# granne/granne

Measured on AMD Instinct MI355X. Metric: queries/sec (recall@10 alongside), 10M x 100-d angular, batch=1024, higher is better.
Workload: dtype f32; 1 GPU; C2 (BASELINE.json configs[1]): 10000000 x 100-d f32 angular, i.i.d. uniform components, batch=1024, ef_search=50, k=10; n_elements=10000000, dim=100, batch=1024, ef_search=50, k=10

## Files before the change

granne_amd/_lib.py:

```python
import ctypes as C
import os

from . import build as _build

F32, I8, F16 = 0, 1, 2
UNUSED = 0xFFFFFFFF
BUILD_ALL = 0xFFFFFFFFFFFFFFFF

OK = 0
ERR_INVALID, ERR_HIP, ERR_NO_DEVICE, ERR_OVERFLOW, ERR_IO = -1, -2, -3, -4, -5

OPT_VISITED_SLOTS, OPT_FORCE_SLOW, OPT_SLOW_SLOTS, OPT_SLOW_BLOCKS, OPT_OVERFLOW_SLOTS = 1, 2, 3, 4, 5
OPT_VISITED16, OPT_VISITED16_LG, OPT_LAST_WALKER, OPT_SEARCH_DEPTH, OPT_INLINE_TAILS, OPT_SEEN_MIN = 6, 7, 8, 9, 10, 11
OPT_SKETCH = 12
OPT_COALESCE, OPT_COALESCE_MAX, OPT_COALESCE_WAIT_US, OPT_COALESCED_LAUNCHES, OPT_COALESCED_QUERIES = 13, 14, 15, 16, 17
OPT_LAST_COMPACT_ROWS = 18
OPT_LAST_SPLIT_TAIL = 19
OPT_LAST_SCAN = 20
OPT_FORCE_GENERAL = 21
(SCAN_NONE, SCAN_RING, SCAN_I8, SCAN_I8_CHUNKED, SCAN_B16_7_4, SCAN_B16_13_2, SCAN_B16_16_1, SCAN_B16_CHUNKED, SCAN_F32_52_4,
 SCAN_F32_100_2, SCAN_F32_128_1) = range(11)
EXACT_TOPK_KMAX = 1024
EXACT_TOPK_CAP = 4096
PF_MAX_STAGES = 8
# ... 54 lines not shown
    "granne_hip_index_create": (i32, [C.POINTER(vp), vp, u64, u32, i32, u32, vp, vp, vp, i32]),
    "granne_hip_index_create_csr": (i32, [C.POINTER(vp), vp, u64, u32, i32, u32, vp, vp, vp, i32]),
    "granne_hip_index_create_device": (i32, [C.POINTER(vp), vp, u64, u32, i32, u32, vp, vp, vp, i32, vp]),
    "granne_hip_index_destroy": (None, [vp]),
    "granne_hip_index_len": (u64, [vp]),
    "granne_hip_index_num_elements": (u64, [vp]),
    "granne_hip_index_num_layers": (u32, [vp]),
    "granne_hip_index_layer_len": (u64, [vp, u32]),
    "granne_hip_index_dim": (u32, [vp]),
    "granne_hip_index_dtype": (i32, [vp]),
    "granne_hip_index_device": (i32, [vp]),
    "granne_hip_index_hbm_bytes": (u64, [vp]),
    "granne_hip_index_get_neighbors": (i32, [vp, u64, u32, vp, u32, C.POINTER(u32)]),
    "granne_hip_index_get_element": (i32, [vp, u64, vp]),
    "granne_hip_index_get_sketch": (i32, [vp, u64, u64, vp]),
    "granne_hip_search_batch": (i32, [vp, vp, u32, u32, u32, vp, vp, vp, vp]),
    "granne_hip_search_batch_device": (i32, [vp, vp, u32, u32, u32, vp, vp, vp, vp, vp, vp]),
    "granne_hip_search_batches_device": (i32, [vp, u32, vp, u32, u32, u32, vp, vp, vp, vp, vp, vp]),
    "granne_hip_search_begin_device": (i32, [vp, vp, u32, u32, u32, vp, vp, vp, vp, vp, vp, C.POINTER(u64)]),
    "granne_hip_search_end_device": (i32, [vp, u64, vp]),
    "granne_hip_device_malloc": (i32, [C.POINTER(vp), u64, i32]),
    "granne_hip_device_free": (i32, [vp, i32]),
    "granne_hip_copy_to_device": (i32, [vp, vp, u64, i32, vp]),
    "granne_hip_copy_to_host": (i32, [vp, vp, u64, i32, vp]),
    "granne_hip_stream_create": (i32, [C.POINTER(vp), i32]),
    "granne_hip_stream_destroy": (i32, [vp, i32]),
    "granne_hip_stream_synchronize": (i32, [vp, i32]),
    "granne_hip_event_create": (i32, [vp]),
    "granne_hip_event_destroy": (None, [vp]),
    "granne_hip_event_elapsed_ms": (i32, [vp, vp, vp]),
# ... 171 lines not shown
```

granne_amd/csrc/brute_force.h:

```cpp
#pragma once

#include "util_kernels.h"

namespace granne_hip {

typedef float bf_f32x16 __attribute__((ext_vector_type(16)));
typedef int bf_i32x16 __attribute__((ext_vector_type(16)));
typedef int bf_i32x4 __attribute__((ext_vector_type(4)));

#ifndef GRANNE_BF_EXP
#define GRANNE_BF_EXP 0
#endif
#ifndef GRANNE_BF_SUB
#define GRANNE_BF_SUB 2
#endif
constexpr uint32_t BF_I8_SUB = GRANNE_BF_SUB;
constexpr uint32_t BF_QT = 256;
constexpr uint32_t BF_THREADS = 512;
constexpr uint32_t BF_EXTRA = 6;
constexpr uint32_t BF_KMAX = 16;

struct BfGeometry {
    uint32_t rows, qt, threads, lds;
};
// ... 1 lines not shown
struct BruteParams {
    const uint8_t* elements;
    uint64_t n;
    uint32_t row_bytes, row_stride, dim;
    const uint8_t* queries;
    uint32_t nq, kk;
    uint64_t per_range;
    uint64_t* part_ids;
    float* part_d;
    uint32_t* part_c;
    const float* inv_norm;
    const float* inv_gmax;
    const float* tau_in;
    uint32_t* share_hist;
    const uint8_t* qpad;
};

struct BfBlock { uint32_t qt, range; };
__device__ __forceinline__ BfBlock bf_block() {
    const uint32_t nqt = gridDim.x, G = gridDim.y;
    const uint32_t L = blockIdx.y * nqt + blockIdx.x;
    BfBlock b;
    if ((G & 7u) == 0u) {
        const uint32_t xcd = L & 7u, slot = L >> 3;
        b.range = xcd * (G >> 3) + slot / nqt;
        b.qt = slot % nqt;
    } else {
        b.qt = blockIdx.x;
        b.range = blockIdx.y;
    }
// ... 223 lines not shown
    if constexpr (PRIME) bf_write_max(P, best, blk.range, q, qlive, h);
    else bf_write_list(P, L, blk.range, q, qlive, h);
}

template <int KH, int R>
constexpr BfGeometry bf_f32_geometry() {
    constexpr uint32_t ET = 32u * R, STRIDE = 2u * KH + 4u;
    return {ET, BF_QT, BF_THREADS, ET * STRIDE * 4u};
}

typedef __bf16 bf_b16x8 __attribute__((ext_vector_type(8)));
typedef __bf16 bf_b16x4 __attribute__((ext_vector_type(4)));
#ifndef GRANNE_BF_B16_AHEAD
#define GRANNE_BF_B16_AHEAD 1
#endif
constexpr uint32_t BF_B16_THREADS = 512, BF_B16_QT = 256;
template <int KG, int R, bool PRIME = false>
__global__ __launch_bounds__(BF_B16_THREADS) void bf_b16_kernel(const BruteParams P) {
    extern __shared__ __align__(16) uint8_t smem_bf[];
    constexpr uint32_t ET = 32u * R;
    constexpr uint32_t COMPS = 16u * KG;
    constexpr uint32_t STRIDE_B = 2u * COMPS + 16u;
    uint8_t* tile_hi = smem_bf;
    uint8_t* tile_lo = smem_bf + (size_t)ET * STRIDE_B;
    const uint32_t tid = threadIdx.x, lane = tid & 63u, wave = tid >> 6;
    const uint32_t col = lane & 31u, h = lane >> 5;
    const BfBlock blk = bf_block();
    const uint32_t q = blk.qt * BF_B16_QT + wave * 32u + col;
    const bool qlive = q < P.nq;

    bf_b16x8 qh[KG], ql[KG];
// ... 939 lines not shown
__global__ void inv_gmax_kernel(const float* __restrict__ inv_norm, uint64_t n, float* __restrict__ out) {
    const uint64_t total = ((n + 31u) >> 5) * 2u;
    for (uint64_t t = (uint64_t)blockIdx.x * blockDim.x + threadIdx.x; t < total; t += (uint64_t)gridDim.x * blockDim.x) {
        const uint64_t b = t >> 1;
        const uint32_t h = (uint32_t)(t & 1u);
        float m = 0.0f;
        for (uint32_t g = 0; g < 4; ++g)
            for (uint32_t i = 0; i < 4; ++i) {
                const uint64_t row = b * 32u + 8u * g + 4u * h + i;
                if (row < n) m = __builtin_fmaxf(m, inv_norm[row]);
            }
        out[t] = m;
    }
}

__global__ __launch_bounds__(64) void bf_tau_kernel(const float* __restrict__ maxima, uint32_t ranges, uint32_t nq, uint32_t kk, float* __restrict__ tau) {
    const uint32_t q = blockIdx.x, lane = threadIdx.x;
    if (q >= nq) return;
    if (ranges < kk || ranges > 64u) {
        if (lane == 0u) tau[q] = -3.0e38f;
        return;
    }
    const float v = lane < ranges ? maxima[(size_t)lane * nq + q] : -3.0e38f;
    uint32_t rank = 0;
    for (uint32_t j = 0; j < ranges; ++j) {
        const float o = __uint_as_float((uint32_t)__builtin_amdgcn_readlane((int)__float_as_uint(v), (int)j));
        rank += (o > v || (o == v && j < lane)) ? 1u : 0u;
    }
    if (lane < ranges && rank + 1u == kk) tau[q] = v > -1.0e38f ? v - 2.0e-6f : -3.0e38f;
}
// ... 43 lines not shown
```

granne_amd/csrc/granne_hip.hip:

```cpp
#include <hip/hip_runtime.h>

#include <atomic>
#include <chrono>
#include <cstdarg>
#include <cstdio>
#include <cstdlib>
#include <cstring>
#include <memory>
#include <mutex>
#include <string>
#include <type_traits>
#include <vector>

#include "../../include/granne_hip.h"
#include "search_kernel.h"
#include "walk_fast.h"
#include "slow_kernel.h"
#include "util_kernels.h"
#include "brute_force.h"
#include "exact_topk.h"
#include "combiner.h"
#include "dev_mem.h"

using namespace granne_hip;
// ... 45 lines not shown
extern "C" const char* granne_hip_last_error(void) { return g_last_error.c_str(); }
extern "C" int granne_hip_abi_version(void) { return GRANNE_HIP_ABI_VERSION; }
extern "C" int granne_hip_device_count(int* out_count) {
    if (!out_count) return fail(GRANNE_HIP_ERR_INVALID, "out_count is null");
    int n = 0;
    hipError_t e = hipGetDeviceCount(&n);
    if (e != hipSuccess) {
        *out_count = 0;
        return fail(GRANNE_HIP_ERR_NO_DEVICE, "hipGetDeviceCount: %s", hipGetErrorString(e));
    }
    *out_count = n;
    return GRANNE_HIP_OK;
}

struct EnvKnobs {
    int visited = 0, touch_max = -1, inline_tails = 1, seen_min = -1, bf_b16 = 1, bf_ring = 1, sketch = 1, compact_rows = 1;
    EnvKnobs() {
        auto geti = [](const char* name, int dflt) {
            const char* e = getenv(name);
            return e ? atoi(e) : dflt;
        };
        visited = geti("GRANNE_HIP_VISITED", 0);
        inline_tails = geti("GRANNE_HIP_INLINE_TAILS", 1);
        bf_ring = geti("GRANNE_HIP_BF_RING", 1);
        bf_b16 = geti("GRANNE_HIP_BF_B16", 1);
        seen_min = geti("GRANNE_HIP_SEEN_MIN", -1);
        touch_max = geti("GRANNE_HIP_TOUCH_MAX", -1);
        compact_rows = geti("GRANNE_HIP_COMPACT_ROWS", 1);
        sketch = geti("GRANNE_HIP_SKETCH", 1);
    }
};
static const EnvKnobs& knobs() {
    static const EnvKnobs k;
    return k;
}

struct ScratchCache {
    struct Block {
        hipStream_t stream;
        DevBuf p;
// ... 52 lines not shown
    uint64_t opt_slow_slots = 1u << 18;
    uint64_t opt_slow_blocks = 16;
    uint64_t opt_overflow_slots = 0;
    uint64_t opt_visited16 = 0;
    uint64_t opt_visited16_lg = 0;
    uint64_t opt_inline_tails = 1;
    uint64_t opt_seen_min = 2048;
    uint64_t opt_sketch = 1;
    std::atomic<uint64_t> last_slow_count{0};
    std::atomic<uint64_t> last_walker{0};
    std::atomic<uint64_t> last_compact{0};
    std::atomic<uint64_t> last_split{0};
    std::atomic<uint64_t> last_scan{0};
    std::mutex norm_mu;
    DevBuf d_inv_norm;
    DevBuf d_sketch;
    struct HostCall {
        hipStream_t stream = nullptr;
        DevBuf d_buf;
        PinBuf h_pin;
    };
    std::mutex call_mu;
    std::vector<HostCall*> call_free;
    uint64_t opt_coalesce = 0;
    Combiner combiner;
    HostCall* group_call[Combiner::DEPTH] = {};
    ScratchCache scratch;
    struct Flight {
        hipStream_t stream = nullptr;
        hipEvent_t ready = nullptr, done = nullptr;
// ... 425 lines not shown
    if (ix->se) return se_rows_to_host(*ix->se, idx, 1, 1, (float*)out);
    DeviceGuard g(ix->device);
    HIP_TRY(hipMemcpy(out, ix->d_elements.as<uint8_t>() + idx * ix->row_stride, (size_t)ix->dim * elem_size(ix->dtype),
                      hipMemcpyDeviceToHost));
    return GRANNE_HIP_OK;
}

extern "C" int granne_hip_index_get_sketch(const granne_hip_index* ix, uint64_t first, uint64_t count, void* out) {
    if (!ix || (!out && count)) return fail(GRANNE_HIP_ERR_INVALID, "null argument");
    GRANNE_HIP_COMPACT_UNSUPPORTED(ix, "get_sketch");
    if (!ix->d_sketch) return fail(GRANNE_HIP_ERR_INVALID, "the index holds no row sketches");
    if (first > ix->n_elements || count > ix->n_elements - first) return fail(GRANNE_HIP_ERR_INVALID, "rows out of range");
    if (count == 0) return GRANNE_HIP_OK;
    DeviceGuard g(ix->device);
    HIP_TRY(hipMemcpy(out, ix->d_sketch.as<uint8_t>() + first * SKETCH_LINE, (size_t)count * SKETCH_LINE, hipMemcpyDeviceToHost));
    return GRANNE_HIP_OK;
}

extern "C" int granne_hip_index_set_option(granne_hip_index* ix, int option, uint64_t value) {
    if (!ix) return fail(GRANNE_HIP_ERR_INVALID, "index is null");
    switch (option) {
    case GRANNE_HIP_OPT_VISITED_SLOTS:
        {
            const uint64_t odd = value ? value >> __builtin_ctzll(value) : 1;
            if (value != 0 && (value < 256 || value > 32768 || (odd != 1 && odd != 3)))
                return fail(GRANNE_HIP_ERR_INVALID, "visited slots must be 0, 2^k or 3 * 2^k in [256, 32768]");
        }
        ix->opt_visited_slots = value;
        return GRANNE_HIP_OK;
    case GRANNE_HIP_OPT_FORCE_SLOW:
// ... 1184 lines not shown
    if (nq && m == 0) return GRANNE_HIP_OK;
    return dists_launch(ix, d_queries, nullptr, m ? m : 1, d_ids, (uint64_t)nq * m, d_out, d_status, stream);
}

static int merge_launch(const uint8_t* ids, const uint8_t* dists, const uint8_t* counts, uint64_t ids_stride,
                        uint64_t dists_stride, uint64_t counts_stride, const uint64_t* shard_offsets, uint32_t n_shards,
                        uint32_t nq, uint32_t k, uint64_t* d_out_ids, float* d_out_dists, uint32_t* d_out_counts,
                        int device_id, void* stream);

struct ScanPlan {
    uint64_t form;
    void (*fn)(const BruteParams);
    void (*prime)(const BruteParams);
    BfGeometry geo, prime_geo;
    uint64_t max_ranges = 64;
};
static ScanPlan plan_scan(const granne_hip_index* ix, uint32_t nq) {
    if (ix->dtype == GRANNE_HIP_I8) {
        if (ix->row_bytes > 128u)
            return {GRANNE_HIP_SCAN_I8_CHUNKED, bf_i8_chunked_kernel<4>, bf_i8_chunked_kernel<4, true>, bf_i8_chunked_geometry<4>(), bf_i8_chunked_geometry<4>()};
        if (knobs().bf_ring && ix->row_bytes == 128u && ix->row_stride == 128u && ix->n_elements < (1ull << 29)) {
            ScanPlan P{GRANNE_HIP_SCAN_RING, bf_i8_ring_kernel, bf_i8_kernel<4, true>, bf_ring_geometry(), bf_i8_geometry<4>()};
            if ((uint64_t)((nq + P.geo.qt - 1) / P.geo.qt) * 64u < 256u) P.max_ranges = 128;
            return P;
        }
        return {GRANNE_HIP_SCAN_I8, bf_i8_kernel<4>, bf_i8_kernel<4, true>, bf_i8_geometry<4>(), bf_i8_geometry<4>()};
    }
    if (knobs().bf_b16 && ix->dim <= 112) return {GRANNE_HIP_SCAN_B16_7_4, bf_b16_kernel<7, 4>, bf_b16_kernel<7, 4, true>, bf_b16_geometry<7, 4>(), bf_b16_geometry<7, 4>()};
    if (knobs().bf_b16 && ix->dim <= 208) return {GRANNE_HIP_SCAN_B16_13_2, bf_b16_kernel<13, 2>, bf_b16_kernel<13, 2, true>, bf_b16_geometry<13, 2>(), bf_b16_geometry<13, 2>()};
    if (ix->dim > 256) return {GRANNE_HIP_SCAN_B16_CHUNKED, bf_b16_chunked_kernel<2>, bf_b16_chunked_kernel<2, true>, bf_b16_chunked_geometry<2>(), bf_b16_chunked_geometry<2>()};
    if (knobs().bf_b16) return {GRANNE_HIP_SCAN_B16_16_1, bf_b16_kernel<16, 1>, bf_b16_kernel<16, 1, true>, bf_b16_geometry<16, 1>(), bf_b16_geometry<16, 1>()};
    if (ix->dim <= 104) return {GRANNE_HIP_SCAN_F32_52_4, bf_f32_kernel<52, 4>, bf_f32_kernel<52, 4, true>, bf_f32_geometry<52, 4>(), bf_f32_geometry<52, 4>()};
    if (ix->dim <= 200) return {GRANNE_HIP_SCAN_F32_100_2, bf_f32_kernel<100, 2>, bf_f32_kernel<100, 2, true>, bf_f32_geometry<100, 2>(), bf_f32_geometry<100, 2>()};
    return {GRANNE_HIP_SCAN_F32_128_1, bf_f32_kernel<128, 1>, bf_f32_kernel<128, 1, true>, bf_f32_geometry<128, 1>(), bf_f32_geometry<128, 1>()};
}

namespace {
struct ScanScratch {
    size_t pid, pd, pc, mid, md, mc, cand, ex, tau, share, qpad, total = 0;
    ScanScratch(uint64_t ranges, uint32_t nq, uint32_t kk, size_t share_bytes, size_t qpad_bytes) {
        auto take = [&](size_t bytes, size_t align) {
            total = (total + align - 1) & ~(align - 1);
            total += bytes;
// ... 84 lines not shown
        std::lock_guard<std::mutex> lk(mix->norm_mu);
        if (!mix->d_inv_norm) {
            DevBuf norms;
            HIP_TRY(norms.alloc((size_t)inv_norm_bytes(n)));
            float* dn = norms.as<float>();
            hipLaunchKernelGGL(inv_norm_rows_kernel, dim3(grid_for(n * 8, 256)), dim3(256), 0, s, ix->d_elements.as<uint8_t>(), n, ix->row_stride, dn);
            hipLaunchKernelGGL(inv_gmax_kernel, dim3(grid_for(n_pad / 16 + 1, 256)), dim3(256), 0, s, (const float*)dn, n, dn + n_pad);
            if (hipGetLastError() != hipSuccess || hipStreamSynchronize(s) != hipSuccess)
                return fail(GRANNE_HIP_ERR_HIP, "inv_norm_rows_kernel failed");
            mix->d_inv_norm = std::move(norms);
            mix->hbm_bytes += inv_norm_bytes(n);
        }
        P.inv_norm = mix->d_inv_norm.as<float>();
        P.inv_gmax = P.inv_norm + n_pad;
    }
    P.elements = ix->d_elements.as<uint8_t>();
    P.n = n;
    P.row_bytes = ix->row_bytes;
    P.row_stride = ix->row_stride;
    P.dim = ix->dim;
    P.queries = (const uint8_t*)d_queries;
    P.nq = nq;
    P.kk = kk;
    P.per_range = per_range;
    P.part_ids = (uint64_t*)(scratch + o.pid);
    P.part_d = (float*)(scratch + o.pd);
    P.part_c = (uint32_t*)(scratch + o.pc);
    if (S.geo.lds > 64u * 1024u) HIP_TRY(hipFuncSetAttribute((const void*)S.fn, hipFuncAttributeMaxDynamicSharedMemorySize, (int)S.geo.lds));
    P.tau_in = nullptr;
    P.share_hist = nullptr;
    P.qpad = nullptr;
    if (qpad_bytes) {
        hipLaunchKernelGGL(bf_pad_queries_kernel, dim3(grid_for(qpad_bytes, 256)), dim3(256), 0, s, (const uint8_t*)d_queries, nq, ix->dim,
                           ix->row_bytes, scratch + o.qpad);
        HIP_TRY(hipGetLastError());
        P.qpad = scratch + o.qpad;
    }
    if (primed) {
        BruteParams Q = P;
        Q.n = prime_n;
        Q.per_range = prime_per;
        const BfGeometry& pg = S.prime_geo;
        if (pg.lds > 64u * 1024u) HIP_TRY(hipFuncSetAttribute((const void*)S.prime, hipFuncAttributeMaxDynamicSharedMemorySize, (int)pg.lds));
        hipLaunchKernelGGL(S.prime, dim3((nq + pg.qt - 1) / pg.qt, (uint32_t)Gs), dim3(pg.threads), pg.lds, s, Q);
        HIP_TRY(hipGetLastError());
        hipLaunchKernelGGL(bf_tau_kernel, dim3(nq), dim3(64), 0, s, (const float*)P.part_d, (uint32_t)Gs, nq, kk, (float*)(scratch + o.tau));
        HIP_TRY(hipGetLastError());
        P.tau_in = (const float*)(scratch + o.tau);
        HIP_TRY(hipMemsetAsync(scratch + o.share, 0, share_bytes, s));
        P.share_hist = (uint32_t*)(scratch + o.share);
    }
    hipLaunchKernelGGL(S.fn, dim3((nq + S.geo.qt - 1) / S.geo.qt, (uint32_t)G), dim3(S.geo.threads), S.geo.lds, s, P);
    HIP_TRY(hipGetLastError());
    int rc = merge_ranges(P, (uint32_t)G, nq, kk, (uint64_t*)(scratch + o.mid), (float*)(scratch + o.md), (uint32_t*)(scratch + o.mc),
                          ix->device, stream);
    if (rc) return rc;
    const uint32_t pairs = nq * kk;
    hipLaunchKernelGGL(bf_narrow_ids_kernel, dim3((pairs + 255) / 256), dim3(256), 0, s, (const uint64_t*)(scratch + o.mid),
                       (const uint32_t*)(scratch + o.mc), nq, kk, (uint32_t*)(scratch + o.cand));
    HIP_TRY(hipGetLastError());
    rc = dists_launch(ix, d_queries, nullptr, kk, (const uint32_t*)(scratch + o.cand), (uint64_t)pairs, (float*)(scratch + o.ex),
                      nullptr, stream);
    if (rc) return rc;
    hipLaunchKernelGGL(bf_final_kernel, dim3((pairs + 255) / 256), dim3(256), 0, s, (const uint32_t*)(scratch + o.cand),
                       (const float*)(scratch + o.ex), nq, kk, k, d_out_ids, d_out_dists, d_out_counts);
    HIP_TRY(hipGetLastError());
    return GRANNE_HIP_OK;
// ... 207 lines not shown
```

granne_amd/csrc/reorder_host.h:

```cpp
#pragma once

#include <hipcub/hipcub.hpp>

namespace granne_hip {

__global__ void iota_u32_kernel(uint32_t* out, uint64_t n, uint32_t first) {
    for (uint64_t t = (uint64_t)blockIdx.x * blockDim.x + threadIdx.x; t < n; t += (uint64_t)gridDim.x * blockDim.x)
        out[t] = first + (uint32_t)t;
}

__global__ void trail_keys_kernel(const uint32_t* __restrict__ trail, const uint32_t* __restrict__ perm,
                                  const uint32_t* __restrict__ order_inv, uint64_t n, uint32_t lo, uint32_t c,
                                  uint64_t* __restrict__ keys) {
    for (uint64_t t = (uint64_t)blockIdx.x * blockDim.x + threadIdx.x; t < n; t += (uint64_t)gridDim.x * blockDim.x) {
        const uint32_t* row = trail + (size_t)(perm[t] - lo) * TRAIL_WIDTH;
        keys[t] = ((uint64_t)order_inv[row[c]] << 32) | (uint64_t)order_inv[row[c + 1]];
    }
}

__global__ void scatter_inverse_kernel(const uint32_t* __restrict__ order, uint64_t n, uint32_t lo,
                                       uint32_t* __restrict__ inv) {
    for (uint64_t t = (uint64_t)blockIdx.x * blockDim.x + threadIdx.x; t < n; t += (uint64_t)gridDim.x * blockDim.x)
        inv[order[t]] = lo + (uint32_t)t;
}
// ... 95 lines not shown
    HIP_TRY(new_el.alloc((size_t)n * ix->row_stride));
    if (n) {
        hipLaunchKernelGGL(permute_rows_kernel, dim3(grid_for(n * (ix->row_stride >> 4), 256)), dim3(256), 0, s,
                           ix->d_elements.as<uint8_t>(), new_el.as<uint8_t>(), d_order, n, ix->row_stride);
        HIP_TRY(hipGetLastError());
    }
    HIP_TRY(hipStreamSynchronize(s));
    for (size_t l = 0; l < ix->layers.size(); ++l) ix->layers[l].d_adj = std::move(new_adj[l]);
    ix->d_elements = std::move(new_el);
    {
        std::lock_guard<std::mutex> lk(ix->norm_mu);
        if (ix->d_inv_norm) {
            ix->d_inv_norm.reset();
            ix->hbm_bytes -= inv_norm_bytes(ix->n_elements);
        }
    }
    return finish_layers(ix, s);
}

static int reorder_precheck(granne_hip_index* ix) {
    if (!ix) return fail(GRANNE_HIP_ERR_INVALID, "index is null");
    GRANNE_HIP_COMPACT_UNSUPPORTED(ix, "reorder");
    GRANNE_HIP_F16_UNSUPPORTED(ix->dtype, "reorder");
    if (ix->layers.empty()) return fail(GRANNE_HIP_ERR_INVALID, "reorder of an index without layers (the reference panics)");
    if (ix->layers.back().len != ix->n_elements)
        return fail(GRANNE_HIP_ERR_INVALID,
                    "reorder needs len() == number of elements (the reference asserts, src/slice_vector/mod.rs:438)");
    return GRANNE_HIP_OK;
}

// ... 131 lines not shown
```

granne_amd/index.py:

```python
import ctypes as C
import os

import numpy as np

from ._lib import ERR_INVALID, ERR_OVERFLOW, EXACT_TOPK_CAP, F16, F32, I8, RANGE_CAP_MAX, GranneHipError, check, lib

DEFAULT_MAX_SEARCH = 200
DEFAULT_NUM_ELEMENTS = 10
RANGE_DEFAULT_STAGES = (252, 1020)

_ELEMENT_TYPES = {"angular": (F32, np.float32), "angular_int": (I8, np.int8), "angular_f16": (F16, np.float16)}
EMBEDDINGS = "embeddings"


def _p(a):
    return a.ctypes.data_as(C.c_void_p)


def normalize(rows, device=0):
    a = np.array(rows, dtype=np.float32, order="C", copy=True)
    flat = a.reshape(1, -1) if a.ndim == 1 else a
    if flat.size:
        check(lib().granne_hip_normalize_f32(_p(flat), flat.shape[0], flat.shape[1], device))
    return a
# ... 263 lines not shown
        check(lib().granne_hip_index_get_neighbors(self._h, idx, layer, _p(buf), buf.size, C.byref(n)))
        return buf[: n.value].astype(np.int64).tolist()

    def get_element(self, idx):
        out = np.empty(self.dim, self.np_dtype)
        check(lib().granne_hip_index_get_element(self._h, idx, _p(out)))
        return out

    def hbm_bytes(self):
        return int(lib().granne_hip_index_hbm_bytes(self._h))

    def get_sketch(self, first=0, count=None):
        count = len(self) - first if count is None else count
        out = np.empty((count, 128), np.uint8)
        if lib().granne_hip_index_get_sketch(self._h, first, count, _p(out)) != 0:
            return None
        return out

    def reorder(self):
        order = np.empty(len(self), np.uint64)
        check(lib().granne_hip_index_reorder(self._h, _p(order)))
        return order

    def reorder_by_keys(self, keys):
        k = np.ascontiguousarray(keys, dtype=np.uint64)
        if k.shape != (len(self),):
            raise ValueError("need one key per element")
        order = np.empty(len(self), np.uint64)
        check(lib().granne_hip_index_reorder_by_keys(self._h, _p(k), _p(order)))
        return order
# ... 492 lines not shown
```

include/granne.hpp:

```cpp
#pragma once

#include <algorithm>
#include <cmath>
#include <cstdint>
#include <cstring>
#include <memory>
#include <stdexcept>
#include <string>
#include <utility>
#include <vector>

#include <type_traits>

#include "granne_hip.h"

namespace granne {

inline void check(int rc) {
    if (rc != GRANNE_HIP_OK) throw std::runtime_error(std::string("granne_hip: ") + granne_hip_last_error());
}

struct f16 {
    uint16_t bits;
};
// ... 451 lines not shown
    void set_coalesce_max(uint64_t queries) { check(granne_hip_index_set_option(h_.get(), GRANNE_HIP_OPT_COALESCE_MAX, queries)); }
    void set_coalesce_wait_us(uint64_t us) { check(granne_hip_index_set_option(h_.get(), GRANNE_HIP_OPT_COALESCE_WAIT_US, us)); }
    uint64_t coalesced_launches() const { return get_option(GRANNE_HIP_OPT_COALESCED_LAUNCHES); }
    uint64_t coalesced_queries() const { return get_option(GRANNE_HIP_OPT_COALESCED_QUERIES); }
    bool last_compact_rows() const { return get_option(GRANNE_HIP_OPT_LAST_COMPACT_ROWS) != 0; }
    bool last_split_tail() const { return get_option(GRANNE_HIP_OPT_LAST_SPLIT_TAIL) != 0; }
    struct LastScan {
        unsigned form, ranges, prime_ranges, kk;
        bool primed;
    };
    LastScan last_scan() const {
        const uint64_t w = get_option(GRANNE_HIP_OPT_LAST_SCAN);
        return {GRANNE_HIP_LAST_SCAN_FORM(w), GRANNE_HIP_LAST_SCAN_RANGES(w), GRANNE_HIP_LAST_SCAN_PRIME_RANGES(w),
                GRANNE_HIP_LAST_SCAN_KK(w), GRANNE_HIP_LAST_SCAN_PRIMED(w) != 0};
    }
    uint64_t get_option(int option) const {
        uint64_t v = 0;
        check(granne_hip_index_get_option(h_.get(), option, &v));
        return v;
    }
    granne_hip_index* raw() const { return h_.get(); }

private:
    static constexpr int dtype() { return detail::dtype_of<typename decltype(Element::data)::value_type>::value; }
    template <class Call>
    std::vector<std::vector<std::pair<size_t, float>>> range_call(const Element* elements, size_t nq, const float* radii, size_t cap,
                                                                  std::vector<uint32_t>* out_found, std::vector<uint32_t>* out_stage,
                                                                  const char* overflow, Call call) const {
        const size_t dim = granne_hip_index_dim(h_.get());
        const int device = granne_hip_index_device(h_.get());
// ... 439 lines not shown
```

include/granne_hip.h:

```cpp
#ifndef GRANNE_HIP_H
#define GRANNE_HIP_H

#include <stddef.h>
#include <stdint.h>

#ifdef __cplusplus
extern "C" {
#endif

#define GRANNE_HIP_ABI_VERSION 3

enum { GRANNE_HIP_F32 = 0, GRANNE_HIP_I8 = 1, GRANNE_HIP_F16 = 2 };

enum {
    GRANNE_HIP_OK = 0,
    GRANNE_HIP_ERR_INVALID = -1,
    GRANNE_HIP_ERR_HIP = -2,
    GRANNE_HIP_ERR_NO_DEVICE = -3,
    GRANNE_HIP_ERR_OVERFLOW = -4,
    GRANNE_HIP_ERR_IO = -5
};

#define GRANNE_HIP_UNUSED 0xFFFFFFFFu

// ... 20 lines not shown

void granne_hip_index_destroy(granne_hip_index* index);

uint64_t granne_hip_index_len(const granne_hip_index* index);
uint64_t granne_hip_index_num_elements(const granne_hip_index* index);
uint32_t granne_hip_index_num_layers(const granne_hip_index* index);
uint64_t granne_hip_index_layer_len(const granne_hip_index* index, uint32_t layer);
uint32_t granne_hip_index_dim(const granne_hip_index* index);
int granne_hip_index_dtype(const granne_hip_index* index);
int granne_hip_index_device(const granne_hip_index* index);
uint64_t granne_hip_index_hbm_bytes(const granne_hip_index* index);
int granne_hip_index_get_neighbors(const granne_hip_index* index, uint64_t node, uint32_t layer,
                                   uint32_t* out_ids, uint32_t cap, uint32_t* out_count);
int granne_hip_index_get_element(const granne_hip_index* index, uint64_t idx, void* out);
int granne_hip_index_get_sketch(const granne_hip_index* index, uint64_t first, uint64_t count, void* out);

int granne_hip_search_batch(const granne_hip_index* index, const void* queries, uint32_t nq,
                            uint32_t max_search, uint32_t num_neighbors, uint64_t* out_ids,
                            float* out_dists, uint32_t* out_counts, uint64_t* out_stats);

int granne_hip_search_batch_device(const granne_hip_index* index, const void* d_queries, uint32_t nq,
                                   uint32_t max_search, uint32_t num_neighbors, uint64_t* d_out_ids,
                                   float* d_out_dists, uint32_t* d_out_counts, uint64_t* d_out_stats,
                                   uint32_t* d_status, void* stream);

int granne_hip_search_batches_device(const granne_hip_index* index, uint32_t n_batches,
                                     const void* const* d_queries, uint32_t nq, uint32_t max_search,
                                     uint32_t num_neighbors, uint64_t* const* d_out_ids,
                                     float* const* d_out_dists, uint32_t* const* d_out_counts,
                                     uint64_t* const* d_out_stats, uint32_t* d_status, void* stream);
// ... 454 lines not shown
```

rust/granne-hip/src/gpu.rs:

```rust
use crate::{angular, angular_int, Index};
use std::marker::PhantomData;
use std::os::raw::{c_char, c_int, c_void};

#[repr(C)] pub struct granne_hip_index { _private: [u8; 0] }
#[repr(C)] pub struct granne_hip_builder { _private: [u8; 0] }
#[repr(C)] pub struct granne_hip_sharded { _private: [u8; 0] }
#[repr(C)] pub struct granne_hip_sum_embeddings { _private: [u8; 0] }
#[repr(C)] pub struct granne_hip_rw_builder { _private: [u8; 0] }

pub const GRANNE_HIP_F32: c_int = 0;
pub const GRANNE_HIP_I8: c_int = 1;
pub const GRANNE_HIP_F16: c_int = 2;
pub const GRANNE_HIP_BUILD_ALL: u64 = u64::MAX;

#[repr(C)]
pub struct granne_hip_build_config {
    pub layer_multiplier: f32,
    pub expected_num_elements: u64,
    pub num_neighbors: u32,
    pub max_search: u32,
    pub reinsert_elements: c_int,
    pub show_progress: c_int,
    pub batch_max: u32,
    pub batch_div: u32,
// ... 22 lines not shown
    fn granne_hip_index_load_on_device(out: *mut *mut granne_hip_index, index_bytes: *const c_void, index_len: u64,
        elements_bytes: *const c_void, elements_len: u64, dtype: c_int, device_id: c_int, staging_bytes: u64,
        out_info: *mut u64) -> c_int;
    fn granne_hip_index_load_files_on_device(out: *mut *mut granne_hip_index, index_path: *const c_char,
        elements_path: *const c_char, dtype: c_int, device_id: c_int, staging_bytes: u64, out_info: *mut u64) -> c_int;
    fn granne_hip_index_destroy(index: *mut granne_hip_index);
    fn granne_hip_index_len(index: *const granne_hip_index) -> u64;
    fn granne_hip_index_num_elements(index: *const granne_hip_index) -> u64;
    fn granne_hip_index_num_layers(index: *const granne_hip_index) -> u32;
    fn granne_hip_index_layer_len(index: *const granne_hip_index, layer: u32) -> u64;
    fn granne_hip_index_dim(index: *const granne_hip_index) -> u32;
    fn granne_hip_index_get_neighbors(index: *const granne_hip_index, node: u64, layer: u32,
        out_ids: *mut u32, cap: u32, out_count: *mut u32) -> c_int;
    fn granne_hip_index_get_element(index: *const granne_hip_index, idx: u64, out: *mut c_void) -> c_int;
    fn granne_hip_index_get_sketch(index: *const granne_hip_index, first: u64, count: u64, out: *mut c_void) -> c_int;
    fn granne_hip_search(index: *const granne_hip_index, query: *const c_void, max_search: u32,
        num_neighbors: u32, out_ids: *mut u64, out_dists: *mut f32, out_count: *mut u32) -> c_int;
    fn granne_hip_search_batch(index: *const granne_hip_index, queries: *const c_void, nq: u32,
        max_search: u32, num_neighbors: u32, out_ids: *mut u64, out_dists: *mut f32,
        out_counts: *mut u32, out_stats: *mut u64) -> c_int;
    fn granne_hip_refine_device(refine_index: *const granne_hip_index, d_queries: *const c_void, nq: u32,
        d_cand_ids: *const u64, d_cand_counts: *const u32, m: u32, k: u32, d_out_ids: *mut u64,
        d_out_dists: *mut f32, d_out_counts: *mut u32, d_refine_status: *mut u32, stream: *mut c_void) -> c_int;
    fn granne_hip_search_refined_batch_device(walk_index: *const granne_hip_index,
        refine_index: *const granne_hip_index, d_walk_queries: *const c_void, d_refine_queries: *const c_void,
        nq: u32, max_search: u32, refine_from: u32, k: u32, d_out_ids: *mut u64, d_out_dists: *mut f32,
        d_out_counts: *mut u32, d_out_stats: *mut u64, d_status: *mut u32, d_refine_status: *mut u32,
        stream: *mut c_void) -> c_int;
    fn granne_hip_search_refined_batch(walk_index: *const granne_hip_index, refine_index: *const granne_hip_index,
        walk_queries: *const c_void, refine_queries: *const c_void, nq: u32, max_search: u32, refine_from: u32,
// ... 1121 lines not shown
```

Measured before the change: 16.41 million queries/s.

## Cache pre-split bf16 scan tiles in HBM and stream them via LDS DMA

On the first brute-force scan, the f32 element rows are converted into a resident image of pre-split bf16 hi/lo tiles laid out exactly as the LDS tile. A new scan kernel then streams whole images into double-buffered LDS with direct DMA, skipping the per-scan f32-to-bf16 split and relayout. It also software-pipelines the LDS fragment reads ahead of the MFMA chain. The cost is extra HBM for the tile image (about the size of the f32 data), a one-time build on first use, and double the LDS per block, which may lower occupancy.

Result: no change. 16.38 million queries/s (-0.2%).

```diff
diff --git a/granne_amd/_lib.py b/granne_amd/_lib.py
--- a/granne_amd/_lib.py
+++ b/granne_amd/_lib.py
@@ -92,6 +92,8 @@
     "granne_hip_index_get_neighbors": (i32, [vp, u64, u32, vp, u32, C.POINTER(u32)]),
     "granne_hip_index_get_element": (i32, [vp, u64, vp]),
     "granne_hip_index_get_sketch": (i32, [vp, u64, u64, vp]),
+    "granne_hip_index_scan_tiles_info": (i32, [vp, vp, vp]),
+    "granne_hip_index_get_scan_tiles": (i32, [vp, u64, u64, vp]),
     "granne_hip_search_batch": (i32, [vp, vp, u32, u32, u32, vp, vp, vp, vp]),
     "granne_hip_search_batch_device": (i32, [vp, vp, u32, u32, u32, vp, vp, vp, vp, vp, vp]),
     "granne_hip_search_batches_device": (i32, [vp, u32, vp, u32, u32, u32, vp, vp, vp, vp, vp, vp]),
diff --git a/granne_amd/csrc/brute_force.h b/granne_amd/csrc/brute_force.h
--- a/granne_amd/csrc/brute_force.h
+++ b/granne_amd/csrc/brute_force.h
@@ -39,6 +39,7 @@
     const float* tau_in;
     uint32_t* share_hist;
     const uint8_t* qpad;
+    const uint8_t* tiles = nullptr;
 };
 
 struct BfBlock { uint32_t qt, range; };
@@ -292,7 +293,85 @@
 #ifndef GRANNE_BF_B16_AHEAD
 #define GRANNE_BF_B16_AHEAD 1
 #endif
+#ifndef GRANNE_BF_B16_TILES_AHEAD
+#define GRANNE_BF_B16_TILES_AHEAD 2
+#endif
 constexpr uint32_t BF_B16_THREADS = 512, BF_B16_QT = 256;
+template <int KG, int R, bool PRIME, int AHEAD, int KK>
+__device__ __forceinline__ void bf_b16_score_tile(const uint8_t* tile_hi, const uint8_t* tile_lo, const bf_b16x8 (&qh)[KG], const bf_b16x8 (&ql)[KG],
+                                                  uint64_t e0, uint64_t r1, uint32_t col, uint32_t h, BfList<KK>& L, float& tau, float& best) {
+    constexpr uint32_t ET = 32u * R, STRIDE_B = 2u * 16u * KG + 16u;
+    bf_f32x16 acc[R];
+#pragma unroll
+    for (int r = 0; r < R; ++r)
+#pragma unroll
+        for (int v = 0; v < 16; ++v) acc[r][v] = 0.0f;
+    const size_t off0 = (size_t)col * STRIDE_B + (size_t)h * 16u * KG;
+    constexpr int NF = KG * R;
+    bf_b16x8 ah[AHEAD + 1], al[AHEAD + 1];
+#pragma unroll
+    for (int i = 0; i < AHEAD && i < NF; ++i) {
+        ah[i] = *reinterpret_cast<const bf_b16x8*>(tile_hi + off0 + (size_t)(i % R) * 32u * STRIDE_B + (size_t)(i / R) * 16u);
+        al[i] = *reinterpret_cast<const bf_b16x8*>(tile_lo + off0 + (size_t)(i % R) * 32u * STRIDE_B + (size_t)(i / R) * 16u);
+    }
+#pragma unroll
+    for (int i = 0; i < NF; ++i) {
+        const int g = i / R, r = i % R;
+        if (i + AHEAD < NF) {
+            const int gn = (i + AHEAD) / R, rn = (i + AHEAD) % R;
+            ah[(i + AHEAD) % (AHEAD + 1)] = *reinterpret_cast<const bf_b16x8*>(tile_hi + off0 + (size_t)rn * 32u * STRIDE_B + (size_t)gn * 16u);
+            al[(i + AHEAD) % (AHEAD + 1)] = *reinterpret_cast<const bf_b16x8*>(tile_lo + off0 + (size_t)rn * 32u * STRIDE_B + (size_t)gn * 16u);
+        }
+        __builtin_amdgcn_sched_barrier(0);
+        acc[r] = __builtin_amdgcn_mfma_f32_32x32x16_bf16(ah[i % (AHEAD + 1)], qh[g], acc[r], 0, 0, 0);
+        acc[r] = __builtin_amdgcn_mfma_f32_32x32x16_bf16(ah[i % (AHEAD + 1)], ql[g], acc[r], 0, 0, 0);
+        acc[r] = __builtin_amdgcn_mfma_f32_32x32x16_bf16(al[i % (AHEAD + 1)], qh[g], acc[r], 0, 0, 0);
+        __builtin_amdgcn_sched_barrier(0);
+    }
+    const bool whole = e0 + ET <= r1;
+#pragma unroll
+    for (int r = 0; r < R; ++r) {
+        if constexpr (PRIME) {
+#pragma unroll
+            for (int v = 0; v < 16; ++v) {
+                const uint64_t e = e0 + (uint32_t)(r * 32 + 8 * (v / 4) + v % 4) + 4u * h;
+                best = (whole || e < r1) ? __builtin_fmaxf(best, acc[r][v]) : best;
+            }
+            continue;
+        }
+        float mx = acc[r][0];
+#pragma unroll
+        for (int v = 1; v < 16; ++v) mx = __builtin_fmaxf(mx, acc[r][v]);
+        if (__ballot(mx > tau)) {
+#pragma unroll
+            for (int v = 0; v < 16; ++v) {
+                const float sc = acc[r][v];
+                const uint64_t e = e0 + (uint32_t)(r * 32 + 8 * (v / 4) + v % 4) + 4u * h;
+                if (sc > tau && (whole || e < r1)) {
+                    L.insert(sc, (uint32_t)e);
+                    tau = __builtin_fmaxf(tau, L.worst());
+                }
+            }
+        }
+    }
+}
+
+template <int KG>
+__device__ __forceinline__ void bf_b16_load_query(const BruteParams& P, uint32_t q, bool qlive, uint32_t h, bf_b16x8 (&qh)[KG], bf_b16x8 (&ql)[KG]) {
+    const float* qp = reinterpret_cast<const float*>(P.queries) + (size_t)(qlive ? q : 0u) * P.dim;
+#pragma unroll
+    for (int g = 0; g < KG; ++g) {
+#pragma unroll
+        for (int j = 0; j < 8; ++j) {
+            const uint32_t c = h * 8u * KG + (uint32_t)g * 8u + (uint32_t)j;
+            const float v = (qlive && c < P.dim) ? qp[c] : 0.0f;
+            const __bf16 hi = (__bf16)v;
+            qh[g][j] = hi;
+            ql[g][j] = (__bf16)(v - (float)hi);
+        }
+    }
+}
+
 template <int KG, int R, bool PRIME = false>
 __global__ __launch_bounds__(BF_B16_THREADS) void bf_b16_kernel(const BruteParams P) {
     extern __shared__ __align__(16) uint8_t smem_bf[];
@@ -1262,6 +1341,95 @@
     }
 }
 
+template <int KG, int R>
+struct BfTiles {
+    static constexpr uint32_t ET = 32u * R, COMPS = 16u * KG, STRIDE_B = 2u * COMPS + 16u;
+    static constexpr uint32_t UNITS = STRIDE_B / 16u;
+    static constexpr uint32_t PIECE = ET * STRIDE_B, IMAGE = 2u * PIECE;
+    static constexpr uint32_t DMAS = IMAGE / 1024u;
+    static constexpr uint32_t DMAS_PER_WAVE = (DMAS + BF_B16_THREADS / 64u - 1u) / (BF_B16_THREADS / 64u);
+    static_assert(UNITS == 2u * KG + 1u && IMAGE % 1024u == 0u, "an image is a whole number of wave transfers");
+    static_assert(2u * IMAGE <= 160u * 1024u, "two images fit a CU's LDS");
+    static constexpr uint64_t bytes(uint64_t n) { return (n + ET - 1u) / ET * IMAGE; }
+};
+
+template <int KG, int R>
+__global__ void scan_tiles_kernel(const uint8_t* __restrict__ elements, uint64_t n, uint32_t row_bytes, uint32_t row_stride, uint8_t* __restrict__ out) {
+    using T = BfTiles<KG, R>;
+    const uint64_t total = (n + T::ET - 1u) / T::ET * T::ET * T::UNITS;
+    const uint32_t row_f4 = row_bytes / 16u;
+    for (uint64_t u = (uint64_t)blockIdx.x * blockDim.x + threadIdx.x; u < total; u += (uint64_t)gridDim.x * blockDim.x) {
+        const uint64_t row = u / T::UNITS;
+        const uint32_t g = (uint32_t)(u - row * T::UNITS);
+        float4 a = make_float4(0.0f, 0.0f, 0.0f, 0.0f), b = a;
+        if (row < n && g < 2u * KG) {
+            const uint8_t* src = elements + row * row_stride;
+            if (2u * g < row_f4) a = *reinterpret_cast<const float4*>(src + (size_t)(2u * g) * 16u);
+            if (2u * g + 1u < row_f4) b = *reinterpret_cast<const float4*>(src + (size_t)(2u * g + 1u) * 16u);
+        }
+        const float v[8] = {a.x, a.y, a.z, a.w, b.x, b.y, b.z, b.w};
+        bf_b16x8 hi, lo;
+#pragma unroll
+        for (int t = 0; t < 8; ++t) {
+            hi[t] = (__bf16)v[t];
+            lo[t] = (__bf16)(v[t] - (float)hi[t]);
+        }
+        uint8_t* dst = out + row / T::ET * T::IMAGE + (row % T::ET) * T::STRIDE_B + g * 16u;
+        *reinterpret_cast<bf_b16x8*>(dst) = hi;
+        *reinterpret_cast<bf_b16x8*>(dst + T::PIECE) = lo;
+    }
+}
+
+template <int KG, int R, bool PRIME = false>
+__global__ __launch_bounds__(BF_B16_THREADS) void bf_b16_tiles_kernel(const BruteParams P) {
+    using T = BfTiles<KG, R>;
+    extern __shared__ __align__(16) uint8_t smem_bf[];
+    const uint32_t tid = threadIdx.x, lane = tid & 63u;
+    const uint32_t wave = (uint32_t)__builtin_amdgcn_readfirstlane((int)(tid >> 6));
+    const uint32_t col = lane & 31u, h = lane >> 5;
+    const BfBlock blk = bf_block();
+    const uint32_t q = blk.qt * BF_B16_QT + wave * 32u + col;
+    const bool qlive = q < P.nq;
+    bf_b16x8 qh[KG], ql[KG];
+    bf_b16_load_query<KG>(P, q, qlive, h, qh, ql);
+    BfList<PRIME ? 1 : BF_KMAX> L;
+    L.init();
+    float tau = bf_start_tau(P, q, qlive);
+    [[maybe_unused]] float best = -3.0e38f;
+
+    const uint64_t r0 = (uint64_t)blk.range * P.per_range;
+    const uint64_t r1 = r0 + P.per_range < P.n ? r0 + P.per_range : P.n;
+    const uint32_t lds0 = (uint32_t)(uintptr_t)smem_bf;
+    auto issue = [&](uint64_t e0, uint32_t slot) {
+        const uint64_t at = (uint64_t)(uintptr_t)P.tiles + e0 / T::ET * T::IMAGE;
+        const uint8_t* img = reinterpret_cast<const uint8_t*>((uint64_t)(uint32_t)__builtin_amdgcn_readfirstlane((int)(uint32_t)at) |
+                                                              (uint64_t)(uint32_t)__builtin_amdgcn_readfirstlane((int)(uint32_t)(at >> 32)) << 32);
+        const uint32_t dst = (uint32_t)__builtin_amdgcn_readfirstlane((int)(lds0 + slot * T::IMAGE));
+#pragma unroll
+        for (uint32_t j = 0; j < T::DMAS_PER_WAVE; ++j) {
+            const uint32_t i = wave + (BF_B16_THREADS / 64u) * j;
+            if (i < T::DMAS) bf_dma16(dst + i * 1024u, img, i * 1024u + lane * 16u);
+        }
+    };
+    if (r0 < r1) issue(r0, 0u);
+    uint32_t slot = 0;
+    for (uint64_t e0 = r0; e0 < r1; e0 += T::ET) {
+        asm volatile("s_waitcnt vmcnt(0)" ::: "memory");
+        __syncthreads();
+        if (e0 + T::ET < r1) issue(e0 + T::ET, slot ^ 1u);
+        const uint8_t* tile_hi = smem_bf + slot * T::IMAGE;
+        bf_b16_score_tile<KG, R, PRIME, GRANNE_BF_B16_TILES_AHEAD>(tile_hi, tile_hi + T::PIECE, qh, ql, e0, r1, col, h, L, tau, best);
+        slot ^= 1u;
+    }
+    if constexpr (PRIME) bf_write_max(P, best, blk.range, q, qlive, h);
+    else bf_write_list(P, L, blk.range, q, qlive, h);
+}
+
+template <int KG, int R>
+constexpr BfGeometry bf_b16_tiles_geometry() {
+    return {BfTiles<KG, R>::ET, BF_B16_QT, BF_B16_THREADS, 2u * BfTiles<KG, R>::IMAGE};
+}
+
 __global__ __launch_bounds__(64) void bf_tau_kernel(const float* __restrict__ maxima, uint32_t ranges, uint32_t nq, uint32_t kk, float* __restrict__ tau) {
     const uint32_t q = blockIdx.x, lane = threadIdx.x;
     if (q >= nq) return;
diff --git a/granne_amd/csrc/granne_hip.hip b/granne_amd/csrc/granne_hip.hip
--- a/granne_amd/csrc/granne_hip.hip
+++ b/granne_amd/csrc/granne_hip.hip
@@ -83,7 +83,7 @@
 }
 
 struct EnvKnobs {
-    int visited = 0, touch_max = -1, inline_tails = 1, seen_min = -1, bf_b16 = 1, bf_ring = 1, sketch = 1, compact_rows = 1;
+    int visited = 0, touch_max = -1, inline_tails = 1, seen_min = -1, bf_b16 = 1, bf_ring = 1, bf_pieces = 1, sketch = 1, compact_rows = 1;
     EnvKnobs() {
         auto geti = [](const char* name, int dflt) {
             const char* e = getenv(name);
@@ -93,6 +93,7 @@
         inline_tails = geti("GRANNE_HIP_INLINE_TAILS", 1);
         bf_ring = geti("GRANNE_HIP_BF_RING", 1);
         bf_b16 = geti("GRANNE_HIP_BF_B16", 1);
+        bf_pieces = geti("GRANNE_HIP_BF_PIECES", 1);
         seen_min = geti("GRANNE_HIP_SEEN_MIN", -1);
         touch_max = geti("GRANNE_HIP_TOUCH_MAX", -1);
         compact_rows = geti("GRANNE_HIP_COMPACT_ROWS", 1);
@@ -175,6 +176,10 @@
     std::atomic<uint64_t> last_scan{0};
     std::mutex norm_mu;
     DevBuf d_inv_norm;
+    DevBuf d_scan_tiles;
+    uint64_t scan_tiles_bytes = 0;
+    bool scan_tiles_refused = false;
+    std::atomic<uint64_t> last_scan_tiles{0};
     DevBuf d_sketch;
     struct HostCall {
         hipStream_t stream = nullptr;
@@ -630,6 +635,27 @@
     if (count == 0) return GRANNE_HIP_OK;
     DeviceGuard g(ix->device);
     HIP_TRY(hipMemcpy(out, ix->d_sketch.as<uint8_t>() + first * SKETCH_LINE, (size_t)count * SKETCH_LINE, hipMemcpyDeviceToHost));
+    return GRANNE_HIP_OK;
+}
+
+extern "C" int granne_hip_index_scan_tiles_info(const granne_hip_index* ix, uint64_t* out_bytes, uint64_t* out_last_scan_read_them) {
+    if (!ix) return fail(GRANNE_HIP_ERR_INVALID, "index is null");
+    if (out_bytes) {
+        std::lock_guard<std::mutex> lk(const_cast<granne_hip_index*>(ix)->norm_mu);
+        *out_bytes = ix->d_scan_tiles ? ix->scan_tiles_bytes : 0;
+    }
+    if (out_last_scan_read_them) *out_last_scan_read_them = ix->last_scan_tiles.load();
+    return GRANNE_HIP_OK;
+}
+
+extern "C" int granne_hip_index_get_scan_tiles(const granne_hip_index* ix, uint64_t first, uint64_t count, void* out) {
+    if (!ix || (!out && count)) return fail(GRANNE_HIP_ERR_INVALID, "null argument");
+    std::lock_guard<std::mutex> lk(const_cast<granne_hip_index*>(ix)->norm_mu);
+    if (!ix->d_scan_tiles) return fail(GRANNE_HIP_ERR_INVALID, "the index holds no scan tiles");
+    if (first > ix->scan_tiles_bytes || count > ix->scan_tiles_bytes - first) return fail(GRANNE_HIP_ERR_INVALID, "bytes out of range");
+    if (count == 0) return GRANNE_HIP_OK;
+    DeviceGuard g(ix->device);
+    HIP_TRY(hipMemcpy(out, ix->d_scan_tiles.as<uint8_t>() + first, (size_t)count, hipMemcpyDeviceToHost));
     return GRANNE_HIP_OK;
 }
 
@@ -1844,6 +1870,11 @@
     void (*prime)(const BruteParams);
     BfGeometry geo, prime_geo;
     uint64_t max_ranges = 64;
+    void (*tiles_fn)(const BruteParams) = nullptr;
+    void (*tiles_prime)(const BruteParams) = nullptr;
+    BfGeometry tiles_geo = {};
+    void (*make_tiles)(const uint8_t*, uint64_t, uint32_t, uint32_t, uint8_t*) = nullptr;
+    uint64_t tiles_bytes = 0;
 };
 static ScanPlan plan_scan(const granne_hip_index* ix, uint32_t nq) {
     if (ix->dtype == GRANNE_HIP_I8) {
@@ -1856,7 +1887,9 @@
         }
         return {GRANNE_HIP_SCAN_I8, bf_i8_kernel<4>, bf_i8_kernel<4, true>, bf_i8_geometry<4>(), bf_i8_geometry<4>()};
     }
-    if (knobs().bf_b16 && ix->dim <= 112) return {GRANNE_HIP_SCAN_B16_7_4, bf_b16_kernel<7, 4>, bf_b16_kernel<7, 4, true>, bf_b16_geometry<7, 4>(), bf_b16_geometry<7, 4>()};
+    if (knobs().bf_b16 && ix->dim <= 112)
+        return {GRANNE_HIP_SCAN_B16_7_4, bf_b16_kernel<7, 4>, bf_b16_kernel<7, 4, true>, bf_b16_geometry<7, 4>(), bf_b16_geometry<7, 4>(), 64,
+                bf_b16_tiles_kernel<7, 4>, bf_b16_tiles_kernel<7, 4, true>, bf_b16_tiles_geometry<7, 4>(), scan_tiles_kernel<7, 4>, BfTiles<7, 4>::bytes(ix->n_elements)};
     if (knobs().bf_b16 && ix->dim <= 208) return {GRANNE_HIP_SCAN_B16_13_2, bf_b16_kernel<13, 2>, bf_b16_kernel<13, 2, true>, bf_b16_geometry<13, 2>(), bf_b16_geometry<13, 2>()};
     if (ix->dim > 256) return {GRANNE_HIP_SCAN_B16_CHUNKED, bf_b16_chunked_kernel<2>, bf_b16_chunked_kernel<2, true>, bf_b16_chunked_geometry<2>(), bf_b16_chunked_geometry<2>()};
     if (knobs().bf_b16) return {GRANNE_HIP_SCAN_B16_16_1, bf_b16_kernel<16, 1>, bf_b16_kernel<16, 1, true>, bf_b16_geometry<16, 1>(), bf_b16_geometry<16, 1>()};
@@ -1971,6 +2004,38 @@
         P.inv_norm = mix->d_inv_norm.as<float>();
         P.inv_gmax = P.inv_norm + n_pad;
     }
+    bool resident = false;
+    if (S.tiles_fn && knobs().bf_pieces) {
+        granne_hip_index* mix = const_cast<granne_hip_index*>(ix);
+        std::lock_guard<std::mutex> lk(mix->norm_mu);
+        hipStreamCaptureStatus cap = hipStreamCaptureStatusNone;
+        if (!mix->d_scan_tiles && !mix->scan_tiles_refused && hipStreamIsCapturing(s, &cap) == hipSuccess && cap == hipStreamCaptureStatusNone) {
+            size_t free_b = 0, total_b = 0;
+            DevBuf tiles;
+            if (hipMemGetInfo(&free_b, &total_b) != hipSuccess || (uint64_t)free_b < S.tiles_bytes + total_b / 32u ||
+                tiles.alloc((size_t)S.tiles_bytes) != hipSuccess) {
+                (void)hipGetLastError();
+                mix->scan_tiles_refused = true;
+            } else {
+                hipLaunchKernelGGL(S.make_tiles, dim3(grid_for(S.tiles_bytes / 32u, 256)), dim3(256), 0, s, ix->d_elements.as<uint8_t>(), n,
+                                   ix->row_bytes, ix->row_stride, tiles.as<uint8_t>());
+                if (hipGetLastError() != hipSuccess || hipStreamSynchronize(s) != hipSuccess)
+                    return fail(GRANNE_HIP_ERR_HIP, "scan_tiles_kernel failed");
+                mix->d_scan_tiles = std::move(tiles);
+                mix->scan_tiles_bytes = S.tiles_bytes;
+                mix->hbm_bytes += S.tiles_bytes;
+            }
+        }
+        if (mix->d_scan_tiles) {
+            P.tiles = mix->d_scan_tiles.as<uint8_t>();
+            resident = true;
+        }
+    }
+    const_cast<granne_hip_index*>(ix)->last_scan_tiles.store(resident ? 1 : 0);
+    void (*const scan_fn)(const BruteParams) = resident ? S.tiles_fn : S.fn;
+    void (*const prime_fn)(const BruteParams) = resident ? S.tiles_prime : S.prime;
+    const BfGeometry& scan_geo = resident ? S.tiles_geo : S.geo;
+    const BfGeometry& prime_geo = resident ? S.tiles_geo : S.prime_geo;
     P.elements = ix->d_elements.as<uint8_t>();
     P.n = n;
     P.row_bytes = ix->row_bytes;
@@ -1983,7 +2048,7 @@
     P.part_ids = (uint64_t*)(scratch + o.pid);
     P.part_d = (float*)(scratch + o.pd);
     P.part_c = (uint32_t*)(scratch + o.pc);
-    if (S.geo.lds > 64u * 1024u) HIP_TRY(hipFuncSetAttribute((const void*)S.fn, hipFuncAttributeMaxDynamicSharedMemorySize, (int)S.geo.lds));
+    if (scan_geo.lds > 64u * 1024u) HIP_TRY(hipFuncSetAttribute((const void*)scan_fn, hipFuncAttributeMaxDynamicSharedMemorySize, (int)scan_geo.lds));
     P.tau_in = nullptr;
     P.share_hist = nullptr;
     P.qpad = nullptr;
@@ -1997,9 +2062,9 @@
         BruteParams Q = P;
         Q.n = prime_n;
         Q.per_range = prime_per;
-        const BfGeometry& pg = S.prime_geo;
-        if (pg.lds > 64u * 1024u) HIP_TRY(hipFuncSetAttribute((const void*)S.prime, hipFuncAttributeMaxDynamicSharedMemorySize, (int)pg.lds));
-        hipLaunchKernelGGL(S.prime, dim3((nq + pg.qt - 1) / pg.qt, (uint32_t)Gs), dim3(pg.threads), pg.lds, s, Q);
+        const BfGeometry& pg = prime_geo;
+        if (pg.lds > 64u * 1024u) HIP_TRY(hipFuncSetAttribute((const void*)prime_fn, hipFuncAttributeMaxDynamicSharedMemorySize, (int)pg.lds));
+        hipLaunchKernelGGL(prime_fn, dim3((nq + pg.qt - 1) / pg.qt, (uint32_t)Gs), dim3(pg.threads), pg.lds, s, Q);
         HIP_TRY(hipGetLastError());
         hipLaunchKernelGGL(bf_tau_kernel, dim3(nq), dim3(64), 0, s, (const float*)P.part_d, (uint32_t)Gs, nq, kk, (float*)(scratch + o.tau));
         HIP_TRY(hipGetLastError());
@@ -2007,7 +2072,7 @@
         HIP_TRY(hipMemsetAsync(scratch + o.share, 0, share_bytes, s));
         P.share_hist = (uint32_t*)(scratch + o.share);
     }
-    hipLaunchKernelGGL(S.fn, dim3((nq + S.geo.qt - 1) / S.geo.qt, (uint32_t)G), dim3(S.geo.threads), S.geo.lds, s, P);
+    hipLaunchKernelGGL(scan_fn, dim3((nq + scan_geo.qt - 1) / scan_geo.qt, (uint32_t)G), dim3(scan_geo.threads), scan_geo.lds, s, P);
     HIP_TRY(hipGetLastError());
     int rc = merge_ranges(P, (uint32_t)G, nq, kk, (uint64_t*)(scratch + o.mid), (float*)(scratch + o.md), (uint32_t*)(scratch + o.mc),
                           ix->device, stream);
diff --git a/granne_amd/csrc/reorder_host.h b/granne_amd/csrc/reorder_host.h
--- a/granne_amd/csrc/reorder_host.h
+++ b/granne_amd/csrc/reorder_host.h
@@ -133,6 +133,12 @@
             ix->d_inv_norm.reset();
             ix->hbm_bytes -= inv_norm_bytes(ix->n_elements);
         }
+        if (ix->d_scan_tiles) {
+            ix->d_scan_tiles.reset();
+            ix->hbm_bytes -= ix->scan_tiles_bytes;
+            ix->scan_tiles_bytes = 0;
+        }
+        ix->scan_tiles_refused = false;
     }
     return finish_layers(ix, s);
 }
diff --git a/granne_amd/index.py b/granne_amd/index.py
--- a/granne_amd/index.py
+++ b/granne_amd/index.py
@@ -301,6 +301,18 @@
         count = len(self) - first if count is None else count
         out = np.empty((count, 128), np.uint8)
         if lib().granne_hip_index_get_sketch(self._h, first, count, _p(out)) != 0:
+            return None
+        return out
+
+    def scan_tiles_info(self):
+        b, r = C.c_uint64(0), C.c_uint64(0)
+        check(lib().granne_hip_index_scan_tiles_info(self._h, C.byref(b), C.byref(r)))
+        return int(b.value), int(r.value)
+
+    def get_scan_tiles(self):
+        size = self.scan_tiles_info()[0]
+        out = np.empty(size, np.uint8)
+        if size == 0 or lib().granne_hip_index_get_scan_tiles(self._h, 0, size, _p(out)) != 0:
             return None
         return out
 
diff --git a/include/granne.hpp b/include/granne.hpp
--- a/include/granne.hpp
+++ b/include/granne.hpp
@@ -489,6 +489,16 @@
         return {GRANNE_HIP_LAST_SCAN_FORM(w), GRANNE_HIP_LAST_SCAN_RANGES(w), GRANNE_HIP_LAST_SCAN_PRIME_RANGES(w),
                 GRANNE_HIP_LAST_SCAN_KK(w), GRANNE_HIP_LAST_SCAN_PRIMED(w) != 0};
     }
+    uint64_t scan_tiles_bytes() const {
+        uint64_t v = 0;
+        check(granne_hip_index_scan_tiles_info(h_.get(), &v, nullptr));
+        return v;
+    }
+    bool last_scan_read_tiles() const {
+        uint64_t v = 0;
+        check(granne_hip_index_scan_tiles_info(h_.get(), nullptr, &v));
+        return v != 0;
+    }
     uint64_t get_option(int option) const {
         uint64_t v = 0;
         check(granne_hip_index_get_option(h_.get(), option, &v));
diff --git a/include/granne_hip.h b/include/granne_hip.h
--- a/include/granne_hip.h
+++ b/include/granne_hip.h
@@ -58,6 +58,8 @@
                                    uint32_t* out_ids, uint32_t cap, uint32_t* out_count);
 int granne_hip_index_get_element(const granne_hip_index* index, uint64_t idx, void* out);
 int granne_hip_index_get_sketch(const granne_hip_index* index, uint64_t first, uint64_t count, void* out);
+int granne_hip_index_scan_tiles_info(const granne_hip_index* index, uint64_t* out_bytes, uint64_t* out_last_scan_read_them);
+int granne_hip_index_get_scan_tiles(const granne_hip_index* index, uint64_t first, uint64_t count, void* out);
 
 int granne_hip_search_batch(const granne_hip_index* index, const void* queries, uint32_t nq,
                             uint32_t max_search, uint32_t num_neighbors, uint64_t* out_ids,
diff --git a/rust/granne-hip/src/gpu.rs b/rust/granne-hip/src/gpu.rs
--- a/rust/granne-hip/src/gpu.rs
+++ b/rust/granne-hip/src/gpu.rs
@@ -60,6 +60,9 @@
         out_ids: *mut u32, cap: u32, out_count: *mut u32) -> c_int;
     fn granne_hip_index_get_element(index: *const granne_hip_index, idx: u64, out: *mut c_void) -> c_int;
     fn granne_hip_index_get_sketch(index: *const granne_hip_index, first: u64, count: u64, out: *mut c_void) -> c_int;
+    fn granne_hip_index_scan_tiles_info(index: *const granne_hip_index, out_bytes: *mut u64,
+        out_last_scan_read_them: *mut u64) -> c_int;
+    fn granne_hip_index_get_scan_tiles(index: *const granne_hip_index, first: u64, count: u64, out: *mut c_void) -> c_int;
     fn granne_hip_search(index: *const granne_hip_index, query: *const c_void, max_search: u32,
         num_neighbors: u32, out_ids: *mut u64, out_dists: *mut f32, out_count: *mut u32) -> c_int;
     fn granne_hip_search_batch(index: *const granne_hip_index, queries: *const c_void, nq: u32,
```
